# seceq/zkir

Measured on AMD Instinct MI355X. Metric: trace rows/sec (2^20-cycle fib: execution-trace fill + BabyBear NTT/LDE + Poseidon2 Merkle commitment), higher is better.
Workload: dtype u32 (Baby Bear, 31-bit modular) / u64 trace words

## Files before the change

### zkir_amd/csrc/poseidon2.h

```cpp
#pragma once
#include "babybear.h"

#ifndef P2_RF_UNROLL
#define P2_RF_UNROLL 1
#endif
namespace p2 {

constexpr int T = 12, RF = 8, RP = 22, RATE = 8, DIGEST = 4;

struct Consts {
  uint32_t ext[RF][T];
  uint32_t in[RP];
  uint32_t diag[T];
  uint32_t pre[RF][T];
  uint32_t ext0_s[T];
  uint64_t pre_b[RF][T];
  uint32_t in_scale;
  uint32_t out_scale;
  uint32_t carry;
  int32_t in0_neg;
  int32_t pr_c[RP];
  uint64_t pr_a[RP];
  uint64_t pr_k[T];
};

inline uint64_t splitmix64(uint64_t& s) {
  uint64_t z = (s += 0x9E3779B97F4A7C15ull);
  z = (z ^ (z >> 30)) * 0xBF58476D1CE4E5B9ull;
  z = (z ^ (z >> 27)) * 0x94D049BB133111EBull;
  return z ^ (z >> 31);
}

inline void ext_matrix_inverse(uint32_t inv[T][T]) {
  static const uint32_t M4[4][4] = {{5, 7, 1, 3}, {4, 6, 1, 1}, {1, 3, 5, 7}, {1, 1, 4, 6}};
  uint32_t a[T][2 * T];
  for (int i = 0; i < T; i++)
    for (int j = 0; j < T; j++) {
      a[i][j] = M4[i & 3][j & 3] * ((i >> 2) == (j >> 2) ? 2u : 1u);
      a[i][T + j] = i == j;
    }
  for (int col = 0; col < T; col++) {
    int piv = col;
    while (a[piv][col] == 0) piv++;
    for (int j = 0; j < 2 * T; j++) { const uint32_t t = a[col][j]; a[col][j] = a[piv][j]; a[piv][j] = t; }
    const uint32_t pinv = bb::inv(a[col][col]);
    for (int j = 0; j < 2 * T; j++) a[col][j] = bb::mul(a[col][j], pinv);
    for (int i = 0; i < T; i++) {
      if (i == col || a[i][col] == 0) continue;
      const uint32_t f = a[i][col];
      for (int j = 0; j < 2 * T; j++) a[i][j] = bb::sub(a[i][j], bb::mul(f, a[col][j]));
    }
  }
  for (int i = 0; i < T; i++) for (int j = 0; j < T; j++) inv[i][j] = a[i][T + j];
}

inline void generate(Consts& c) {
  uint64_t s = 0x5A4B49522D50322Dull;
  auto next = [&]() -> uint32_t { for (;;) { const uint32_t v = (uint32_t)(splitmix64(s) >> 33); if (v < bb::P) return bb::to_mont(v); } };
  for (int r = 0; r < RF; r++) for (int i = 0; i < T; i++) c.ext[r][i] = next();
  for (int r = 0; r < RP; r++) c.in[r] = next();
  c.diag[0] = bb::to_mont(bb::P - 2);
  for (int i = 1; i < T; i++) c.diag[i] = bb::to_mont(1u << (i - 1));
  uint32_t minv[T][T];
  ext_matrix_inverse(minv);
  for (int r = 0; r < RF; r++)
    for (int i = 0; i < T; i++) {
      uint32_t v = 0;
      if (r != RF / 2 - 1 && r != RF - 1)
        for (int j = 0; j < T; j++) v = bb::add(v, bb::mul(minv[i][j], bb::from_mont(c.ext[r + 1][j])));
      c.pre[r][i] = bb::to_mont(bb::to_mont(v));
    }
  {
    constexpr uint64_t INV7 = 1725656503ull;
    const uint32_t R = bb::R1, Rinv = bb::inv(R);
    const uint32_t R6 = bb::pow(R, 6);
    uint32_t g[RF + 1], h[RF];
    g[RF / 2] = R;
    for (int r = RF / 2 - 1; r >= 0; r--) { h[r] = bb::mul(g[r + 1], R); g[r] = bb::pow(bb::mul(h[r], R6), INV7); }
    {
      uint32_t f[RP], hx[RP];
      for (int r = 0; r < RP; r++) { f[r] = r < 3 ? R : bb::mul(f[r - 3], Rinv); hx[r] = bb::pow(bb::mul(f[r], R6), INV7); }
      const uint32_t G = bb::mul(f[RP - 1], Rinv), R2c = bb::mul(R, R);
      for (int r = 0; r < RP; r++) {
        const uint32_t hn = r + 1 < RP ? hx[r + 1] : G, rcn = bb::from_mont(r + 1 < RP ? c.in[r + 1] : c.ext[RF / 2][0]);
        c.pr_c[r] = (int32_t)bb::mul(bb::mul(hn, R2c), bb::inv(f[r]));
        c.pr_a[r] = bb::mul(bb::mul(hn, rcn), R);
      }
      c.pr_k[0] = 0;
      for (int i = 1; i < T; i++) c.pr_k[i] = bb::mul(f[RP - 1], bb::from_mont(c.ext[RF / 2][i]));
      g[RF / 2] = G;
    }
    for (int r = RF / 2; r < RF; r++) { h[r] = bb::mul(bb::pow(g[r], 7), bb::inv(R6)); g[r + 1] = bb::mul(h[r], Rinv); }
    const uint32_t f_in = bb::mul(g[0], R), f_out = g[RF];
    for (int i = 0; i < T; i++) c.ext0_s[i] = bb::mul(bb::from_mont(c.ext[0][i]), f_in);
    for (int r = 0; r < RF; r++)
      for (int i = 0; i < T; i++) {
        uint32_t v = 0;
        if (r != RF / 2 - 1 && r != RF - 1)
          for (int j = 0; j < T; j++) v = bb::add(v, bb::mul(minv[i][j], bb::from_mont(c.ext[r + 1][j])));
        c.pre_b[r][i] = ((uint64_t)bb::P << 32) | bb::mul(bb::mul(v, h[r]), R);
      }
    c.in_scale = bb::mul(f_in, R);
    c.out_scale = bb::mul(R, bb::inv(f_out));
    c.carry = bb::mul(bb::mul(f_in, R), bb::inv(f_out));
    c.in0_neg = (int32_t)c.in[0] - (int32_t)bb::P;
  }
}

BB_HD uint32_t sbox_lazy(uint32_t x, uint32_t addend = 0) {
  const uint32_t x2 = bb::mont_mul_lazy(x, x), x3 = bb::mont_mul(x2, x), x6 = bb::mont_mul_lazy(x3, x3);
  return bb::mont_mul_add_lazy(x6, x, addend);
}
BB_HD uint32_t sbox(uint32_t x) { return bb::reduce_2p(sbox_lazy(x)); }

BB_HD void m4_wide(uint32_t a, uint32_t b, uint32_t c, uint32_t d, uint64_t* y) {
#if defined(P2_ZEXT_MAD) && defined(__HIP_DEVICE_COMPILE__)
  uint64_t za, zc;
  asm("v_mad_u64_u32 %0, vcc, %1, 1, 0" : "=v"(za) : "v"(a) : "vcc");
  asm("v_mad_u64_u32 %0, vcc, %1, 1, 0" : "=v"(zc) : "v"(c) : "vcc");
  const uint64_t t0 = bb::mad_wide<1>(za, b), t1 = bb::mad_wide<1>(zc, d);
#else
  const uint64_t t0 = bb::acc_add(a, b), t1 = bb::acc_add(c, d);
#endif
  const uint64_t t2 = bb::mad_wide<2>(t1, b), t3 = bb::mad_wide<2>(t0, d);
  const uint64_t t4 = (t1 << 2) + t3, t5 = (t0 << 2) + t2;
  y[0] = t3 + t5; y[1] = t5; y[2] = t2 + t4; y[3] = t4;
}
template <bool ADD_RC>
BB_HD void ext_linear(uint32_t* s, const uint32_t* rc) {
  uint64_t y[T];
// ... 88 lines not shown
  uint64_t acc = (uint64_t)w[1];
#pragma unroll
  for (int i = 2; i < T; i++) acc += (uint64_t)w[i];
  const int64_t sum = bb::sacc_add((int64_t)acc, s0);
  x = int_next_x(smad<-2>(sum, s0), c, r);
#pragma unroll
  for (int i = 1; i < T; i++) w[i] = (int64_t)(((uint64_t)w[i] << (i - 1)) + (uint64_t)sum);
}
constexpr uint64_t lazy_rounds_bound(uint64_t start, int rounds) {
  uint64_t b[T] = {}, top = 0;
  for (int i = 1; i < T; i++) b[i] = start;
  for (int r = 0; r < rounds; r++) {
    uint64_t sum = bb::P;
    for (int i = 1; i < T; i++) sum += b[i];
    if (sum + 2 * (uint64_t)bb::P > top) top = sum + 2 * (uint64_t)bb::P;
    for (int i = 1; i < T; i++) { b[i] = sum + (b[i] << (i - 1)); if (b[i] > top) top = b[i]; }
  }
  return top;
}
constexpr uint64_t lazy_reduced_bound(uint64_t acc) { return (acc >> 32) + bb::P / 2 + 2; }
static_assert(lazy_rounds_bound(1ull << 31, 3) < (1ull << 62), "three partial rounds on words below 2^31 stay inside what a Montgomery reduction takes");
static_assert(lazy_reduced_bound(lazy_rounds_bound(1ull << 31, 3)) <= (1ull << 31), ".. and their reduction is a word below 2^31 again");
static_assert(lazy_reduced_bound(lazy_rounds_bound(1ull << 31, 1) + bb::P) < bb::P, "the words leave the last round (one round + the next full round's constant) inside (-p, p)");
BB_HD void int_rounds_scaled(uint32_t* s, const Consts& c) {
  int32_t x = (int32_t)s[0] + c.in0_neg;
  int32_t t[T];
  int64_t w[T];
#pragma unroll
  for (int i = 1; i < T; i++) t[i] = (int32_t)s[i];
#pragma unroll 1
  for (int r = 0; r < RP - 1; r += 3) {
    int_round_a(x, t, w, c, r);
    int_round_w(x, w, c, r + 1);
    int_round_w(x, w, c, r + 2);
#pragma unroll
    for (int i = 1; i < T; i++) t[i] = bb::smont_reduce_wide(w[i]);
  }
  int_round_a(x, t, w, c, RP - 1);
  s[0] = (uint32_t)x;
#pragma unroll
  for (int i = 1; i < T; i++) s[i] = (uint32_t)bb::smont_reduce_wide((int64_t)((uint64_t)w[i] + c.pr_k[i]));
}
BB_HD void permute_scaled(uint32_t* s, const Consts& c) {
  ext_linear_scaled<true>(s, c.ext0_s);
#pragma unroll P2_RF_UNROLL
  for (int r = 0; r < RF / 2; r++) {
#pragma unroll
    for (int i = 0; i < T; i++) s[i] = sbox_biased(s[i], c.pre_b[r][i]);
    ext_linear_scaled<false>(s, nullptr);
  }
  int_rounds_scaled(s, c);
#pragma unroll P2_RF_UNROLL
  for (int r = RF / 2; r < RF; r++) {
#pragma unroll
    for (int i = 0; i < T; i++) s[i] = sbox_biased(s[i], c.pre_b[r][i]);
    ext_linear_scaled<false>(s, nullptr);
  }
}

#if defined(__HIPCC__)
template <int CTRL>
__device__ __forceinline__ uint32_t quad_perm(uint32_t v) { return (uint32_t)__builtin_amdgcn_mov_dpp((int)v, CTRL, 0xF, 0xF, true); }
template <int CTRL>
__device__ __forceinline__ uint64_t quad_perm64(uint64_t v) { return ((uint64_t)quad_perm<CTRL>((uint32_t)(v >> 32)) << 32) | quad_perm<CTRL>((uint32_t)v); }

template <bool ADD_RC>
__device__ __forceinline__ void ext_linear_quad_scaled(uint32_t* s, const uint32_t* m4row, const uint32_t* rc) {
  uint64_t y[3];
#pragma unroll
  for (int b = 0; b < 3; b++) {
    const uint32_t v0 = quad_perm<0x00>(s[b]), v1 = quad_perm<0x55>(s[b]), v2 = quad_perm<0xAA>(s[b]), v3 = quad_perm<0xFF>(s[b]);
    y[b] = (uint64_t)v0 * m4row[0] + (uint64_t)v1 * m4row[1] + (uint64_t)v2 * m4row[2] + (uint64_t)v3 * m4row[3];
  }
  const uint64_t sum = y[0] + y[1] + y[2];
#pragma unroll
  for (int b = 0; b < 3; b++) {
    uint64_t v = y[b] + sum;
    if (ADD_RC) v += rc[b];
    s[b] = bb::mont_reduce_wide(v);
  }
// ... 108 lines not shown
```

### zkir_amd/csrc/stark.hip

```cpp
#include <hip/hip_runtime.h>

#include <array>
#include <atomic>
#include <chrono>
#include <cstdio>
#include <cstdlib>
#include <cstddef>
#include <memory>
#include <mutex>
#include <vector>

#include "../../include/zkir_amd.h"
#include "../../include/zkir_amd_experimental.h"
#include "air.h"
#include "babybear.h"
#include "host.h"
#include "hashcall.h"
#include "poseidon2.h"
#include "verify_stages.h"

namespace {

constexpr int NT = 256;

// ... 413 lines not shown
}


__global__ __launch_bounds__(NT) void selector_inverse_kernel(uint32_t log_n, const uint32_t* __restrict__ tw_fwd, uint32_t* __restrict__ inv_xm1) {
  const uint32_t N2 = 2u << log_n, N = N2 >> 1;
  const uint32_t j0 = (blockIdx.x * NT + threadIdx.x) * 8;
  if (j0 >= N2) return;
  uint32_t d[8], pre[8];
  uint32_t run = bb::R1;
#pragma unroll
  for (int k = 0; k < 8; k++) {
    const uint32_t j = j0 + k;
    const uint32_t wj = j < N ? tw_fwd[j] : bb::neg(tw_fwd[j - N]);
    d[k] = bb::sub(bb::mont_mul(wj, bb::to_mont(bb::GEN)), bb::R1);
    pre[k] = run; run = bb::mont_mul(run, d[k]);
  }
  uint32_t inv = bb::R1, b = run, e = bb::P - 2;
  while (e) { if (e & 1) inv = bb::mont_mul(inv, b); b = bb::mont_mul(b, b); e >>= 1; }
#pragma unroll
  for (int k = 7; k >= 0; k--) { inv_xm1[j0 + k] = bb::mont_mul(inv, pre[k]); inv = bb::mont_mul(inv, d[k]); }
}


__global__ __launch_bounds__(NT) void leaf_hash_kernel(const p2::Consts* __restrict__ cp, const uint32_t* __restrict__ mat, uint32_t width, uint64_t n, uint32_t in_scale, uint32_t* __restrict__ digests) {
  const uint64_t j = (uint64_t)blockIdx.x * NT + threadIdx.x;
  if (j >= n) return;
  uint32_t s[p2::T];
#pragma unroll
  for (int i = 0; i < p2::T; i++) s[i] = 0;
  const uint4* m4 = reinterpret_cast<const uint4*>(mat);
  const uint32_t carry = cp->carry, out_scale = cp->out_scale;
  for (uint32_t off = 0; off < width; off += p2::RATE) {
    const uint4 lo = m4[((uint64_t)(off >> 3) * n + j) * 2], hi = m4[((uint64_t)(off >> 3) * n + j) * 2 + 1];
    const uint32_t v[8] = {lo.x, lo.y, lo.z, lo.w, hi.x, hi.y, hi.z, hi.w};
#pragma unroll
    for (int i = 0; i < p2::RATE; i++) s[i] = off + i < width ? bb::mont_mul_lazy(v[i], in_scale) : bb::mont_mul_lazy(s[i], carry);
#pragma unroll
    for (int i = p2::RATE; i < p2::T; i++) s[i] = bb::mont_mul_lazy(s[i], carry);
    p2::permute_scaled(s, *cp);
  }
  if (width == 0) p2::permute_scaled(s, *cp);
  uint4 d = make_uint4(bb::mont_mul(s[0], out_scale), bb::mont_mul(s[1], out_scale), bb::mont_mul(s[2], out_scale), bb::mont_mul(s[3], out_scale));
  reinterpret_cast<uint4*>(digests)[j] = d;
}

__global__ __launch_bounds__(NT) void leaf_absorb_kernel(const p2::Consts* __restrict__ cp, const uint32_t* __restrict__ mat, uint32_t width, uint32_t b0, uint32_t b1, uint64_t n, uint32_t in_scale,
                                                         uint4* __restrict__ state, int first, int last, uint32_t* __restrict__ digests) {
  const uint64_t j = (uint64_t)blockIdx.x * NT + threadIdx.x;
  if (j >= n) return;
  uint32_t s[p2::T];
  if (first) {
#pragma unroll
    for (int i = 0; i < p2::T; i++) s[i] = 0;
  } else {
    const uint4 a = state[j], b = state[n + j], c = state[2 * n + j];
    s[0] = a.x; s[1] = a.y; s[2] = a.z; s[3] = a.w; s[4] = b.x; s[5] = b.y; s[6] = b.z; s[7] = b.w; s[8] = c.x; s[9] = c.y; s[10] = c.z; s[11] = c.w;
  }
  const uint4* m4 = reinterpret_cast<const uint4*>(mat);
  const uint32_t carry = cp->carry, out_scale = cp->out_scale;
  for (uint32_t blk = b0; blk < b1; blk++) {
    const uint32_t off = blk * 8;
    const uint4 lo = m4[((uint64_t)blk * n + j) * 2], hi = m4[((uint64_t)blk * n + j) * 2 + 1];
    const uint32_t v[8] = {lo.x, lo.y, lo.z, lo.w, hi.x, hi.y, hi.z, hi.w};
#pragma unroll
    for (int i = 0; i < p2::RATE; i++) s[i] = off + i < width ? bb::mont_mul_lazy(v[i], in_scale) : bb::mont_mul_lazy(s[i], carry);
#pragma unroll
    for (int i = p2::RATE; i < p2::T; i++) s[i] = bb::mont_mul_lazy(s[i], carry);
    p2::permute_scaled(s, *cp);
  }
  if (last) {
    reinterpret_cast<uint4*>(digests)[j] = make_uint4(bb::mont_mul(s[0], out_scale), bb::mont_mul(s[1], out_scale), bb::mont_mul(s[2], out_scale), bb::mont_mul(s[3], out_scale));
  } else {
    state[j] = make_uint4(s[0], s[1], s[2], s[3]); state[n + j] = make_uint4(s[4], s[5], s[6], s[7]); state[2 * n + j] = make_uint4(s[8], s[9], s[10], s[11]);
  }
}

__global__ __launch_bounds__(NT) void compress_kernel(const p2::Consts* __restrict__ cp, const uint32_t* __restrict__ in, uint64_t n_out, uint32_t* __restrict__ out) {
  const uint64_t i = (uint64_t)blockIdx.x * NT + threadIdx.x;
  if (i >= n_out) return;
  const uint4 l = reinterpret_cast<const uint4*>(in)[2 * i], r = reinterpret_cast<const uint4*>(in)[2 * i + 1];
  const uint32_t k = cp->in_scale, ko = cp->out_scale;
  uint32_t s[p2::T] = {bb::mont_mul_lazy(l.x, k), bb::mont_mul_lazy(l.y, k), bb::mont_mul_lazy(l.z, k), bb::mont_mul_lazy(l.w, k), bb::mont_mul_lazy(r.x, k), bb::mont_mul_lazy(r.y, k),
                       bb::mont_mul_lazy(r.z, k), bb::mont_mul_lazy(r.w, k), 0, 0, 0, 0};
  p2::permute_scaled(s, *cp);
  reinterpret_cast<uint4*>(out)[i] = make_uint4(bb::mont_mul(s[0], ko), bb::mont_mul(s[1], ko), bb::mont_mul(s[2], ko), bb::mont_mul(s[3], ko));
}

constexpr uint32_t SUBTREE = 1024, NT_SUB = 1024;
__global__ __launch_bounds__(NT_SUB) void subtree_kernel(const p2::Consts* __restrict__ cp, uint32_t* cur, uint64_t m, uint32_t per_wg, uint32_t* counter) {
  __shared__ uint4 buf[SUBTREE];
  __shared__ uint32_t last_one;
  const uint32_t t = threadIdx.x;
  uint64_t pos0 = (uint64_t)blockIdx.x * per_wg;
  for (uint32_t e = t; e < per_wg; e += NT_SUB) {
    const uint4 v = reinterpret_cast<const uint4*>(cur)[pos0 + e];
    buf[e] = make_uint4(bb::to_mont(v.x), bb::to_mont(v.y), bb::to_mont(v.z), bb::to_mont(v.w));
  }
  __syncthreads();
 levels:
  for (uint32_t cnt = per_wg; cnt > 1; cnt >>= 1) {
    cur += 4 * m; m >>= 1; pos0 >>= 1;
    const uint32_t n_perm = cnt / 2;
    if (n_perm > NT_SUB / 16) {
      const bool active = t < n_perm;
      uint32_t s[p2::T];
      if (active) {
        const uint4 l = buf[2 * t], r = buf[2 * t + 1];
        const uint32_t k_in = bb::from_mont(cp->in_scale);
        s[0] = bb::mont_mul_lazy(l.x, k_in); s[1] = bb::mont_mul_lazy(l.y, k_in); s[2] = bb::mont_mul_lazy(l.z, k_in); s[3] = bb::mont_mul_lazy(l.w, k_in);
        s[4] = bb::mont_mul_lazy(r.x, k_in); s[5] = bb::mont_mul_lazy(r.y, k_in); s[6] = bb::mont_mul_lazy(r.z, k_in); s[7] = bb::mont_mul_lazy(r.w, k_in);
        s[8] = s[9] = s[10] = s[11] = 0;
      }
      __syncthreads();
      if (active) {
        p2::permute_scaled(s, *cp);
        const uint32_t ko = cp->out_scale, ko_m = bb::to_mont(ko);
        buf[t] = make_uint4(bb::mont_mul(s[0], ko_m), bb::mont_mul(s[1], ko_m), bb::mont_mul(s[2], ko_m), bb::mont_mul(s[3], ko_m));
        reinterpret_cast<uint4*>(cur)[pos0 + t] = make_uint4(bb::mont_mul(s[0], ko), bb::mont_mul(s[1], ko), bb::mont_mul(s[2], ko), bb::mont_mul(s[3], ko));
      }
    } else {
      const uint32_t pi = t >> 4, l = t & 15;
      const bool active = pi < n_perm;
      const uint32_t* words = reinterpret_cast<const uint32_t*>(buf);
      uint32_t s = 0;
      if (active && l < 8) s = bb::mont_mul_lazy(words[8 * pi + l], bb::from_mont(cp->in_scale));
      __syncthreads();
      if (active) {
        s = p2::permute_row16_scaled(s, (int)l, *cp);
        if (l < 4) {
          const uint32_t ko = cp->out_scale;
          reinterpret_cast<uint32_t*>(buf)[4 * pi + l] = bb::mont_mul(s, bb::to_mont(ko));
          cur[4 * (pos0 + pi) + l] = bb::mont_mul(s, ko);
        }
      }
    }
    __syncthreads();
  }
#if defined(__HIP_DEVICE_COMPILE__) && !defined(__gfx950__)
#error "subtree_kernel's hand-over relies on the gfx950 (gfx9) s_waitcnt encoding and on vmcnt covering stores"
#endif
  if (m > 1) {
    if (t < 4) {
      const uint32_t v = reinterpret_cast<const uint32_t*>(buf)[t];
      __hip_atomic_store(&cur[4 * pos0 + t], bb::from_mont(v), __ATOMIC_RELAXED, __HIP_MEMORY_SCOPE_AGENT);
      asm volatile("" ::: "memory");
      __builtin_amdgcn_s_waitcnt(0x0F70);
      asm volatile("" ::: "memory");
    }
    if (t == 0) {
      const uint32_t done = __hip_atomic_fetch_add(counter, 1u, __ATOMIC_RELAXED, __HIP_MEMORY_SCOPE_AGENT);
      asm volatile("" ::: "memory");
      last_one = done == (uint32_t)m - 1;
      if (last_one) __hip_atomic_store(counter, 0u, __ATOMIC_RELAXED, __HIP_MEMORY_SCOPE_AGENT);
    }
    __syncthreads();
    if (!last_one) return;
    asm volatile("" ::: "memory");
    per_wg = (uint32_t)m; pos0 = 0;
    for (uint32_t e = t; e < 4 * per_wg; e += NT_SUB)
      reinterpret_cast<uint32_t*>(buf)[e] = bb::to_mont(__hip_atomic_load(&cur[e], __ATOMIC_RELAXED, __HIP_MEMORY_SCOPE_AGENT));
    __syncthreads();
    goto levels;
  }
}

__global__ __launch_bounds__(NT) void modmul_peak_kernel(uint32_t* __restrict__ out, uint32_t iters) {
  uint32_t a[8], c[8];
#pragma unroll
  for (int k = 0; k < 8; k++) { a[k] = (threadIdx.x * 2654435761u + blockIdx.x * 40503u + k * 7919u) % bb::P; c[k] = (a[k] * 31u + 7u) % bb::P; }
  for (uint32_t i = 0; i < iters; i++) {
#pragma unroll
    for (int k = 0; k < 8; k++) a[k] = bb::mont_mul_lazy(a[k], c[k]);
  }
  uint32_t r = 0;
#pragma unroll
  for (int k = 0; k < 8; k++) r ^= a[k];
  if (r == 0xFFFFFFFFu && iters == 0xFFFFFFFFu) out[0] = r;
}

constexpr uint32_t SYNC_SLOTS = 1024;
struct SyncRing {
  uint32_t* d_slots = nullptr;
  std::atomic<uint32_t> next{0};
// ... 23 lines not shown
  uint32_t* d_g_lo = nullptr;
  uint32_t* d_g_lo_m = nullptr;
  uint32_t* d_inv_xm1 = nullptr;
  uint32_t* d_g_hi = nullptr;
  uint32_t* d_small_inv = nullptr;
  uint32_t* d_small_fwd = nullptr;
  p2::Consts consts;
  p2::Consts* d_p2 = nullptr;
  mutable hipStream_t ov_stream = nullptr; mutable hipEvent_t ov_ev[2] = {nullptr, nullptr}; mutable std::vector<hipEvent_t> ov_group_ev; mutable uint4* d_ov_state = nullptr; mutable size_t ov_state_bytes = 0;
  mutable SyncRing sync;
  mutable std::mutex mu;
  mutable unsigned char* arena = nullptr;
  mutable size_t arena_size = 0, arena_off = 0;
  mutable zkir::HostPin pin;
};

namespace {
int lde_launch(const zkir_stark_ctx* c, uint32_t* in, uint32_t width, uint32_t* out, bool mont_out, hipStream_t s) {
  const zkir::LdeTables t{(int)c->log_n, c->d_tw_inv, c->d_tw_fwd, mont_out ? c->d_g_lo_m : c->d_g_lo, c->d_g_hi, c->d_small_inv, c->d_small_fwd};
  zkir::lde_run(t, in, (width + 7) / 8, out, s);
  return check_launch("lde");
}
int merkle_commit(const zkir_stark_ctx* c, const uint32_t* mat, uint32_t width, uint64_t n_leaves, uint32_t* tree, bool mont_in, hipStream_t s) {
  hipLaunchKernelGGL(leaf_hash_kernel, dim3(grid_for(n_leaves)), dim3(NT), 0, s, c->d_p2, mat, width, n_leaves, mont_in ? bb::from_mont(c->consts.in_scale) : c->consts.in_scale, tree);
  launch_tree_levels(c->d_p2, tree, n_leaves, c->sync, s);
  return check_launch("merkle_commit");
}
}

extern "C" {

uint32_t zkir_main_trace_width(void) { return air::committed_width(false); }
uint32_t zkir_main_trace_width_for(uint32_t deferred) { return air::committed_width((int)deferred); }

void zkir_poseidon2_permute(uint32_t state[12]) {
  static const p2::Consts consts = [] { p2::Consts c; p2::generate(c); return c; }();
  uint32_t s[p2::T];
  for (int i = 0; i < p2::T; i++) s[i] = bb::to_mont(state[i] % bb::P);
  p2::permute(s, consts);
  for (int i = 0; i < p2::T; i++) state[i] = bb::from_mont(s[i]);
}

void zkir_poseidon2_permute_scaled(uint32_t state[12], uint32_t rounds) {
  static const p2::Consts consts = [] { p2::Consts c; p2::generate(c); return c; }();
  uint32_t s[p2::T];
  for (int i = 0; i < p2::T; i++) s[i] = bb::mont_mul_lazy(state[i] % bb::P, consts.in_scale);
  for (uint32_t r = 0; r < rounds; r++) {
// ... 46 lines not shown
  uint32_t* d = nullptr;
  if (hipMalloc(&d, 256) != hipSuccess) return 0.0;
  const uint32_t blocks = 256 * 16, iters = 4096;
  hipEvent_t a, b;
  (void)hipEventCreate(&a); (void)hipEventCreate(&b);
  hipLaunchKernelGGL(modmul_peak_kernel, dim3(blocks), dim3(NT), 0, s, d, 64u);
  (void)hipEventRecord(a, s);
  hipLaunchKernelGGL(modmul_peak_kernel, dim3(blocks), dim3(NT), 0, s, d, iters);
  (void)hipEventRecord(b, s);
  (void)hipEventSynchronize(b);
  float ms = 0;
  (void)hipEventElapsedTime(&ms, a, b);
  (void)hipEventDestroy(a); (void)hipEventDestroy(b); (void)hipFree(d);
  return ms > 0 ? (double)blocks * NT * iters * 8.0 / (ms * 1e-3) : 0.0;
}

int zkir_stark_ctx_create(uint32_t log_n, uint32_t log_blowup, zkir_stark_ctx** out) {
  if (!out || log_n < 1 || log_n > 26 || log_blowup != 1) { zkir::set_last_error({ZKIR_ERR_ARGUMENT, "zkir_stark_ctx_create: need 1 <= log_n <= 26 and log_blowup == 1"}); return ZKIR_ERR_ARGUMENT; }
  *out = nullptr;
  zkir_stark_ctx* c = new zkir_stark_ctx();
  c->log_n = log_n; c->log_blowup = log_blowup;
  const uint32_t N = 1u << log_n;
  const uint32_t n_inv = N >= 2 ? N / 2 : 1, n_hi = (N >> 10) + 1;
  p2::generate(c->consts);
  hipError_t e = hipMalloc((void**)&c->d_p2, sizeof(p2::Consts));
  if (e == hipSuccess) e = hipMemcpy(c->d_p2, &c->consts, sizeof(p2::Consts), hipMemcpyHostToDevice);
  if (e == hipSuccess) e = hipMalloc(&c->sync.d_slots, SYNC_SLOTS * sizeof(uint32_t));
  if (e == hipSuccess) e = hipMemset(c->sync.d_slots, 0, SYNC_SLOTS * sizeof(uint32_t));
  if (e == hipSuccess) e = hipMalloc(&c->d_tw_inv, (size_t)n_inv * 4);
  if (e == hipSuccess) e = hipMalloc(&c->d_tw_fwd, (size_t)N * 4);
  if (e == hipSuccess) e = hipMalloc(&c->d_g_lo, 1024 * 4);
  if (e == hipSuccess) e = hipMalloc(&c->d_g_hi, (size_t)n_hi * 4);
  if (e == hipSuccess) e = hipMalloc(&c->d_g_lo_m, 1024 * 4);
  if (e == hipSuccess) e = hipMalloc(&c->d_inv_xm1, (size_t)2 * N * 4);
  const int Bm = log_n < 10 ? (int)log_n : 10;
  const uint32_t n_si = Bm >= 1 ? (1u << (Bm - 1)) : 1, n_sf = 1u << Bm;
  if (e == hipSuccess) e = hipMalloc(&c->d_small_inv, (size_t)n_si * 4);
  if (e == hipSuccess) e = hipMalloc(&c->d_small_fwd, (size_t)n_sf * 4);
  if (e != hipSuccess) { zkir::set_last_error({ZKIR_ERR_DEVICE, std::string("zkir_stark_ctx_create: ") + hipGetErrorString(e)}); zkir_stark_ctx_free(c); return ZKIR_ERR_DEVICE; }
  const uint32_t wN = bb::root_of_unity(log_n), w2N = bb::root_of_unity(log_n + 1);
  hipLaunchKernelGGL(powers_kernel, dim3(grid_for(n_inv)), dim3(NT), 0, 0, bb::inv(wN), bb::R1, c->d_tw_inv, n_inv);
  hipLaunchKernelGGL(powers_kernel, dim3(grid_for(N)), dim3(NT), 0, 0, w2N, bb::R1, c->d_tw_fwd, N);
  hipLaunchKernelGGL(powers_kernel, dim3(4), dim3(NT), 0, 0, bb::GEN, bb::to_mont(bb::inv(N % bb::P)), c->d_g_lo, 1024u);
  hipLaunchKernelGGL(powers_kernel, dim3(4), dim3(NT), 0, 0, bb::GEN, bb::to_mont(bb::to_mont(bb::inv(N % bb::P))), c->d_g_lo_m, 1024u);
  hipLaunchKernelGGL(powers_kernel, dim3(grid_for(n_hi)), dim3(NT), 0, 0, bb::pow(bb::GEN, 1024), bb::R1, c->d_g_hi, n_hi);
  hipLaunchKernelGGL(selector_inverse_kernel, dim3(grid_for((2ull * N + 7) / 8)), dim3(NT), 0, 0, log_n, c->d_tw_fwd, c->d_inv_xm1);
  hipLaunchKernelGGL(powers_kernel, dim3(grid_for(n_si)), dim3(NT), 0, 0, bb::inv(bb::root_of_unity(Bm)), bb::R1, c->d_small_inv, n_si);
  hipLaunchKernelGGL(powers_kernel, dim3(grid_for(n_sf)), dim3(NT), 0, 0, bb::root_of_unity(Bm + 1), bb::R1, c->d_small_fwd, n_sf);
  if (hipDeviceSynchronize() != hipSuccess || check_launch("stark ctx tables") != ZKIR_OK) { zkir_stark_ctx_free(c); return ZKIR_ERR_DEVICE; }
// ... 137 lines not shown
  const zkir::LdeTables t{(int)c->log_n, c->d_tw_inv, c->d_tw_fwd, c->d_g_lo, c->d_g_hi, c->d_small_inv, c->d_small_fwd};
  (void)hipEventRecord(c->ov_ev[0], s); (void)hipStreamWaitEvent(c->ov_stream, c->ov_ev[0], 0);
  for (uint32_t g = 0; g < n_groups; g++) {
    const uint32_t b0 = g * group, b1 = std::min(nb, b0 + group);
    zkir::lde_run(t, in + (uint64_t)b0 * N * 8, b1 - b0, out + (uint64_t)b0 * N2 * 8, s);
    (void)hipEventRecord(c->ov_group_ev[g], s); (void)hipStreamWaitEvent(c->ov_stream, c->ov_group_ev[g], 0);
    hipLaunchKernelGGL(leaf_absorb_kernel, dim3(grid_for(N2)), dim3(NT), 0, c->ov_stream, c->d_p2, out, width, b0, b1, N2, c->consts.in_scale, c->d_ov_state, g == 0 ? 1 : 0, g + 1 == n_groups ? 1 : 0, tree);
  }
  (void)hipEventRecord(c->ov_ev[1], c->ov_stream); (void)hipStreamWaitEvent(s, c->ov_ev[1], 0);
  launch_tree_levels(c->d_p2, tree, N2, c->sync, s);
  return check_launch("commit_overlapped");
}

int zkir_lde_launch(const zkir_stark_ctx* c, uint32_t* in, uint32_t width, uint32_t* out, void* stream) { return lde_launch(c, in, width, out, false, (hipStream_t)stream); }

int zkir_merkle_commit_launch(const zkir_stark_ctx* c, const uint32_t* mat, uint32_t width, uint64_t n_leaves, uint32_t* tree, void* stream) {
  hipStream_t s = (hipStream_t)stream;
  if (!c || n_leaves == 0 || (n_leaves & (n_leaves - 1))) { zkir::set_last_error({ZKIR_ERR_ARGUMENT, "merkle: null context, or n_leaves not a power of two"}); return ZKIR_ERR_ARGUMENT; }
  return merkle_commit(c, mat, width, n_leaves, tree, false, s);
}

int zkir_merkle_leaves_launch(const zkir_stark_ctx* c, const uint32_t* mat, uint32_t width, uint64_t n_leaves, uint32_t* digests, void* stream) {
  if (!c || !mat || !digests || n_leaves == 0) { zkir::set_last_error({ZKIR_ERR_ARGUMENT, "merkle leaves: null argument or no leaves"}); return ZKIR_ERR_ARGUMENT; }
  hipLaunchKernelGGL(leaf_hash_kernel, dim3(grid_for(n_leaves)), dim3(NT), 0, (hipStream_t)stream, c->d_p2, mat, width, n_leaves, c->consts.in_scale, digests);
  return check_launch("merkle_leaves");
}

int zkir_merkle_cap_launch(const zkir_stark_ctx* c, uint32_t* tree, uint64_t n_digests, void* stream) {
  if (!c || n_digests == 0 || (n_digests & (n_digests - 1))) { zkir::set_last_error({ZKIR_ERR_ARGUMENT, "merkle cap: null context, or n_digests not a power of two"}); return ZKIR_ERR_ARGUMENT; }
  launch_tree_levels(c->d_p2, tree, n_digests, c->sync, (hipStream_t)stream);
  return check_launch("merkle_cap");
}

}

#include "stark_prove.inl"
```

Measured before the change: 196.1 million.

## Fold Poseidon2 input scaling into per-domain constant sets and prune dead sponge lanes

Builds three Poseidon2 constant sets (scaled, canonical-input, Montgomery-input). Each set folds the input scaling into the round constants and the first-round factors, so leaf hashing and compression no longer multiply every input word by a scale. A new sponge path precomputes the capacity lanes for zero-capacity compression, skips the reductions of dead output lanes in the last linear layer, and merges the entry constant of the partial rounds into one multiply-add. It also drops the to_mont/from_mont conversions in the subtree kernel and adds an occupancy hint to the leaf and compress kernels. The cost is three times the device constant memory and more complex constant derivation, which brings a correctness risk.

```diff
diff --git a/zkir_amd/csrc/poseidon2.h b/zkir_amd/csrc/poseidon2.h
--- a/zkir_amd/csrc/poseidon2.h
+++ b/zkir_amd/csrc/poseidon2.h
@@ -22,7 +22,13 @@
   int32_t pr_c[RP];
   uint64_t pr_a[RP];
   uint64_t pr_k[T];
+  int32_t x0_mul;
+  uint64_t x0_add;
+  uint32_t rc_in[T];
+  uint64_t rc_car[T];
+  uint64_t cap0_y[4];
 };
+constexpr int SET_SCALED = 0, SET_CANON = 1, SET_MONT = 2, N_SETS = 3;
 
 inline uint64_t splitmix64(uint64_t& s) {
   uint64_t z = (s += 0x9E3779B97F4A7C15ull);
@@ -54,14 +60,13 @@
   for (int i = 0; i < T; i++) for (int j = 0; j < T; j++) inv[i][j] = a[i][T + j];
 }
 
-inline void generate(Consts& c) {
+inline void generate_rounds(Consts& c, uint32_t minv[T][T]) {
   uint64_t s = 0x5A4B49522D50322Dull;
   auto next = [&]() -> uint32_t { for (;;) { const uint32_t v = (uint32_t)(splitmix64(s) >> 33); if (v < bb::P) return bb::to_mont(v); } };
   for (int r = 0; r < RF; r++) for (int i = 0; i < T; i++) c.ext[r][i] = next();
   for (int r = 0; r < RP; r++) c.in[r] = next();
   c.diag[0] = bb::to_mont(bb::P - 2);
   for (int i = 1; i < T; i++) c.diag[i] = bb::to_mont(1u << (i - 1));
-  uint32_t minv[T][T];
   ext_matrix_inverse(minv);
   for (int r = 0; r < RF; r++)
     for (int i = 0; i < T; i++) {
@@ -70,42 +75,67 @@
         for (int j = 0; j < T; j++) v = bb::add(v, bb::mul(minv[i][j], bb::from_mont(c.ext[r + 1][j])));
       c.pre[r][i] = bb::to_mont(bb::to_mont(v));
     }
+}
+constexpr uint64_t INV7 = 1725656503ull;
+inline void generate_factors(Consts& c, uint32_t f_in, const uint32_t minv[T][T]) {
+  const uint32_t R = bb::R1, Rinv = bb::inv(R);
+  const uint32_t R6 = bb::pow(R, 6), R6inv = bb::inv(R6);
+  uint32_t g[RF + 1], h[RF];
+  g[0] = bb::mul(f_in, Rinv);
+  for (int r = 0; r < RF / 2; r++) { h[r] = bb::mul(bb::pow(g[r], 7), R6inv); g[r + 1] = bb::mul(h[r], Rinv); }
   {
-    constexpr uint64_t INV7 = 1725656503ull;
-    const uint32_t R = bb::R1, Rinv = bb::inv(R);
-    const uint32_t R6 = bb::pow(R, 6);
-    uint32_t g[RF + 1], h[RF];
-    g[RF / 2] = R;
-    for (int r = RF / 2 - 1; r >= 0; r--) { h[r] = bb::mul(g[r + 1], R); g[r] = bb::pow(bb::mul(h[r], R6), INV7); }
-    {
-      uint32_t f[RP], hx[RP];
-      for (int r = 0; r < RP; r++) { f[r] = r < 3 ? R : bb::mul(f[r - 3], Rinv); hx[r] = bb::pow(bb::mul(f[r], R6), INV7); }
-      const uint32_t G = bb::mul(f[RP - 1], Rinv), R2c = bb::mul(R, R);
-      for (int r = 0; r < RP; r++) {
-        const uint32_t hn = r + 1 < RP ? hx[r + 1] : G, rcn = bb::from_mont(r + 1 < RP ? c.in[r + 1] : c.ext[RF / 2][0]);
-        c.pr_c[r] = (int32_t)bb::mul(bb::mul(hn, R2c), bb::inv(f[r]));
-        c.pr_a[r] = bb::mul(bb::mul(hn, rcn), R);
-      }
-      c.pr_k[0] = 0;
-      for (int i = 1; i < T; i++) c.pr_k[i] = bb::mul(f[RP - 1], bb::from_mont(c.ext[RF / 2][i]));
-      g[RF / 2] = G;
-    }
-    for (int r = RF / 2; r < RF; r++) { h[r] = bb::mul(bb::pow(g[r], 7), bb::inv(R6)); g[r + 1] = bb::mul(h[r], Rinv); }
-    const uint32_t f_in = bb::mul(g[0], R), f_out = g[RF];
-    for (int i = 0; i < T; i++) c.ext0_s[i] = bb::mul(bb::from_mont(c.ext[0][i]), f_in);
-    for (int r = 0; r < RF; r++)
-      for (int i = 0; i < T; i++) {
-        uint32_t v = 0;
-        if (r != RF / 2 - 1 && r != RF - 1)
-          for (int j = 0; j < T; j++) v = bb::add(v, bb::mul(minv[i][j], bb::from_mont(c.ext[r + 1][j])));
-        c.pre_b[r][i] = ((uint64_t)bb::P << 32) | bb::mul(bb::mul(v, h[r]), R);
-      }
-    c.in_scale = bb::mul(f_in, R);
-    c.out_scale = bb::mul(R, bb::inv(f_out));
-    c.carry = bb::mul(bb::mul(f_in, R), bb::inv(f_out));
-    c.in0_neg = (int32_t)c.in[0] - (int32_t)bb::P;
-  }
-}
+    uint32_t f[RP], hx[RP];
+    const uint32_t f0 = g[RF / 2];
+    for (int r = 0; r < RP; r++) { f[r] = r < 3 ? f0 : bb::mul(f[r - 3], Rinv); hx[r] = bb::pow(bb::mul(f[r], R6), INV7); }
+    const uint32_t G = bb::mul(f[RP - 1], Rinv), R2c = bb::mul(R, R);
+    for (int r = 0; r < RP; r++) {
+      const uint32_t hn = r + 1 < RP ? hx[r + 1] : G, rcn = bb::from_mont(r + 1 < RP ? c.in[r + 1] : c.ext[RF / 2][0]);
+      c.pr_c[r] = (int32_t)bb::mul(bb::mul(hn, R2c), bb::inv(f[r]));
+      c.pr_a[r] = bb::mul(bb::mul(hn, rcn), R);
+    }
+    c.pr_k[0] = 0;
+    for (int i = 1; i < T; i++) c.pr_k[i] = bb::mul(f[RP - 1], bb::from_mont(c.ext[RF / 2][i]));
+    c.x0_mul = (int32_t)bb::mul(bb::mul(hx[0], R), bb::inv(f0));
+    c.x0_add = bb::mul(bb::mul(hx[0], bb::from_mont(c.in[0])), R);
+    g[RF / 2] = G;
+  }
+  for (int r = RF / 2; r < RF; r++) { h[r] = bb::mul(bb::pow(g[r], 7), R6inv); g[r + 1] = bb::mul(h[r], Rinv); }
+  const uint32_t f_out = g[RF];
+  for (int i = 0; i < T; i++) c.ext0_s[i] = bb::mul(bb::from_mont(c.ext[0][i]), f_in);
+  for (int r = 0; r < RF; r++)
+    for (int i = 0; i < T; i++) {
+      uint32_t v = 0;
+      if (r != RF / 2 - 1 && r != RF - 1)
+        for (int j = 0; j < T; j++) v = bb::add(v, bb::mul(minv[i][j], bb::from_mont(c.ext[r + 1][j])));
+      c.pre_b[r][i] = ((uint64_t)bb::P << 32) | bb::mul(bb::mul(v, h[r]), R);
+    }
+  c.in_scale = bb::mul(f_in, R);
+  c.out_scale = bb::mul(R, bb::inv(f_out));
+  c.carry = bb::mul(bb::mul(f_in, R), bb::inv(f_out));
+  c.in0_neg = (int32_t)c.in[0] - (int32_t)bb::P;
+  for (int i = 0; i < T; i++) {
+    uint32_t v = 0;
+    for (int j = 0; j < T; j++) v = bb::add(v, bb::mul(minv[i][j], bb::from_mont(c.ext[0][j])));
+    c.rc_in[i] = bb::mul(v, f_in);
+    c.rc_car[i] = bb::mul(c.rc_in[i], R);
+  }
+  const uint64_t a = c.rc_in[8], b = c.rc_in[9], cc = c.rc_in[10], d = c.rc_in[11];
+  c.cap0_y[0] = 5 * a + 7 * b + cc + 3 * d; c.cap0_y[1] = 4 * a + 6 * b + cc + d; c.cap0_y[2] = a + 3 * b + 5 * cc + 7 * d; c.cap0_y[3] = a + b + 4 * cc + 6 * d;
+}
+inline void generate(Consts& c) {
+  uint32_t minv[T][T];
+  generate_rounds(c, minv);
+  const uint32_t R = bb::R1, R6 = bb::pow(R, 6);
+  uint32_t g = R;
+  for (int r = RF / 2 - 1; r >= 0; r--) g = bb::pow(bb::mul(bb::mul(g, R), R6), INV7);
+  generate_factors(c, bb::mul(g, R), minv);
+}
+inline void generate_for(Consts& c, uint32_t f_in) {
+  uint32_t minv[T][T];
+  generate_rounds(c, minv);
+  generate_factors(c, f_in, minv);
+}
+inline void generate_sets(Consts* sets) { generate(sets[SET_SCALED]); generate_for(sets[SET_CANON], 1u); generate_for(sets[SET_MONT], bb::R1); }
 
 BB_HD uint32_t sbox_lazy(uint32_t x, uint32_t addend = 0) {
   const uint32_t x2 = bb::mont_mul_lazy(x, x), x3 = bb::mont_mul(x2, x), x6 = bb::mont_mul_lazy(x3, x3);
@@ -240,8 +270,11 @@
 static_assert(lazy_rounds_bound(1ull << 31, 3) < (1ull << 62), "three partial rounds on words below 2^31 stay inside what a Montgomery reduction takes");
 static_assert(lazy_reduced_bound(lazy_rounds_bound(1ull << 31, 3)) <= (1ull << 31), ".. and their reduction is a word below 2^31 again");
 static_assert(lazy_reduced_bound(lazy_rounds_bound(1ull << 31, 1) + bb::P) < bb::P, "the words leave the last round (one round + the next full round's constant) inside (-p, p)");
+static_assert((((uint64_t)bb::P + 128) * bb::P + bb::P) < ((uint64_t)bb::P << 31), "the entry product of word 0 is inside what a signed Montgomery product takes");
+static_assert(((((uint64_t)bb::P + 128) * bb::P + bb::P) >> 32) + bb::P / 2 + 2 < bb::P, ".. and leaves |x| < p, inside the S-box input bound |x| <= p + 128");
+template <bool ENTRY_MUL = false>
 BB_HD void int_rounds_scaled(uint32_t* s, const Consts& c) {
-  int32_t x = (int32_t)s[0] + c.in0_neg;
+  int32_t x = ENTRY_MUL ? bb::smont_mul_add((int32_t)s[0], c.x0_mul, c.x0_add) : (int32_t)s[0] + c.in0_neg;
   int32_t t[T];
   int64_t w[T];
 #pragma unroll
@@ -267,13 +300,133 @@
     for (int i = 0; i < T; i++) s[i] = sbox_biased(s[i], c.pre_b[r][i]);
     ext_linear_scaled<false>(s, nullptr);
   }
-  int_rounds_scaled(s, c);
+  int_rounds_scaled<false>(s, c);
 #pragma unroll P2_RF_UNROLL
   for (int r = RF / 2; r < RF; r++) {
 #pragma unroll
     for (int i = 0; i < T; i++) s[i] = sbox_biased(s[i], c.pre_b[r][i]);
     ext_linear_scaled<false>(s, nullptr);
   }
+}
+
+enum Live { LIVE_ALL, LIVE_CAP, LIVE_DIGEST };
+template <bool ZERO_CAP>
+BB_HD void ext_linear_first(uint32_t* s, const Consts& c) {
+  uint64_t y[T];
+  m4_wide(s[0], s[1], s[2], s[3], y); m4_wide(s[4], s[5], s[6], s[7], y + 4);
+  if (ZERO_CAP) {
+#pragma unroll
+    for (int j = 0; j < 4; j++) y[8 + j] = c.cap0_y[j];
+  } else m4_wide(s[8], s[9], s[10], s[11], y + 8);
+  uint64_t sum[4];
+#pragma unroll
+  for (int j = 0; j < 4; j++) sum[j] = y[j] + y[4 + j] + y[8 + j];
+#pragma unroll
+  for (int k = 0; k < T; k++) s[k] = bb::mont_reduce_wide(y[k] + sum[k & 3]);
+}
+BB_HD void dead4(uint32_t* s) {
+#if defined(__HIP_DEVICE_COMPILE__)
+  asm("" : "=v"(s[0]), "=v"(s[1]), "=v"(s[2]), "=v"(s[3]));
+#else
+  s[0] = s[1] = s[2] = s[3] = 0;
+#endif
+}
+BB_HD Live uniform(Live l) {
+#if defined(__HIP_DEVICE_COMPILE__)
+  uint32_t v = (uint32_t)l;
+  asm("" : "+s"(v));
+  return (Live)v;
+#else
+  return l;
+#endif
+}
+BB_HD void ext_linear_live(uint32_t* s, Live live) {
+  uint64_t y[T];
+  m4_wide(s[0], s[1], s[2], s[3], y); m4_wide(s[4], s[5], s[6], s[7], y + 4); m4_wide(s[8], s[9], s[10], s[11], y + 8);
+  uint64_t sum[4];
+#pragma unroll
+  for (int j = 0; j < 4; j++) sum[j] = y[j] + y[4 + j] + y[8 + j];
+  if (live == LIVE_ALL) {
+#pragma unroll
+    for (int k = 0; k < T; k++) s[k] = bb::mont_reduce_wide(y[k] + sum[k & 3]);
+  } else if (live == LIVE_CAP) {
+#pragma unroll
+    for (int k = RATE; k < T; k++) s[k] = bb::mont_reduce_wide(y[k] + sum[k & 3]);
+    dead4(s); dead4(s + 4);
+  } else {
+#pragma unroll
+    for (int k = 0; k < DIGEST; k++) s[k] = bb::mont_reduce_wide(y[k] + sum[k & 3]);
+    dead4(s + 4); dead4(s + 8);
+  }
+}
+template <bool ZERO_CAP>
+BB_HD void sponge_rounds(uint32_t* s, const Consts& c, Live live) {
+  ext_linear_first<ZERO_CAP>(s, c);
+#pragma unroll P2_RF_UNROLL
+  for (int r = 0; r < RF / 2; r++) {
+#pragma unroll
+    for (int i = 0; i < T; i++) s[i] = sbox_biased(s[i], c.pre_b[r][i]);
+    ext_linear_scaled<false>(s, nullptr);
+  }
+  int_rounds_scaled<true>(s, c);
+#pragma unroll P2_RF_UNROLL
+  for (int r = RF / 2; r < RF; r++) {
+#pragma unroll
+    for (int i = 0; i < T; i++) s[i] = sbox_biased(s[i], c.pre_b[r][i]);
+    ext_linear_live(s, r < RF - 1 ? LIVE_ALL : live);
+  }
+}
+template <Live LIVE, bool ZERO_CAP>
+BB_HD void permute_sponge(uint32_t* s, const Consts& c) { sponge_rounds<ZERO_CAP>(s, c, uniform(LIVE)); }
+BB_HD void sponge_absorb(uint32_t* s, const uint32_t* x, const Consts& c) {
+#pragma unroll
+  for (int i = 0; i < RATE; i++) s[i] = x[i] + c.rc_in[i];
+}
+BB_HD uint32_t sponge_keep(uint32_t s, const Consts& c, int i) { return bb::mont_mul_add_lazy(s, c.carry, c.rc_car[i]); }
+BB_HD const Consts& fresh(const Consts& c) {
+  uint32_t z = 0;
+#if defined(__HIP_DEVICE_COMPILE__)
+  asm volatile("" : "+s"(z));
+#endif
+  return (&c)[z];
+}
+template <class Load>
+BB_HD void sponge_hash(const Consts& c, uint32_t width, Load&& load, uint32_t* digest) {
+  const uint32_t nb = (width + RATE - 1) / RATE, rag = width % RATE;
+  uint32_t s[T];
+  uint32_t b = 0;
+  do {
+    uint32_t v[RATE] = {0, 0, 0, 0, 0, 0, 0, 0};
+    const Consts& k = fresh(c);
+    const bool ragged = rag && b + 1 == nb;
+    if (b < nb) load(b, v);
+    if (b == 0) {
+      const uint32_t n0 = nb == 0 ? 0u : ragged ? rag : (uint32_t)RATE;
+#pragma unroll
+      for (int i = 0; i < RATE; i++) s[i] = ((uint32_t)i < n0 ? v[i] : 0u) + k.rc_in[i];
+#pragma unroll
+      for (int i = RATE; i < T; i++) s[i] = k.rc_in[i];
+    } else {
+      if (ragged) {
+#pragma unroll
+        for (int i = 0; i < RATE; i++) s[i] = (uint32_t)i < rag ? v[i] + k.rc_in[i] : sponge_keep(s[i], k, i);
+      } else sponge_absorb(s, v, k);
+#pragma unroll
+      for (int i = RATE; i < T; i++) s[i] = sponge_keep(s[i], k, i);
+    }
+    sponge_rounds<false>(s, k, b + 1 >= nb ? LIVE_DIGEST : rag && b + 2 == nb ? LIVE_ALL : LIVE_CAP);
+  } while (++b < nb);
+#pragma unroll
+  for (int i = 0; i < DIGEST; i++) digest[i] = bb::mont_mul(s[i], c.out_scale);
+}
+BB_HD void sponge_compress(const Consts& c, const uint32_t* x, uint32_t* digest) {
+  uint32_t s[T];
+  sponge_absorb(s, x, c);
+#pragma unroll
+  for (int i = RATE; i < T; i++) s[i] = 0;
+  permute_sponge<LIVE_DIGEST, true>(s, c);
+#pragma unroll
+  for (int i = 0; i < DIGEST; i++) digest[i] = bb::mont_mul(s[i], c.out_scale);
 }
 
 #if defined(__HIPCC__)
diff --git a/zkir_amd/csrc/stark.hip b/zkir_amd/csrc/stark.hip
--- a/zkir_amd/csrc/stark.hip
+++ b/zkir_amd/csrc/stark.hip
@@ -459,26 +459,17 @@
 }
 
 
-__global__ __launch_bounds__(NT) void leaf_hash_kernel(const p2::Consts* __restrict__ cp, const uint32_t* __restrict__ mat, uint32_t width, uint64_t n, uint32_t in_scale, uint32_t* __restrict__ digests) {
+constexpr int P2_WAVES = 8;
+__global__ __launch_bounds__(NT, P2_WAVES) void leaf_hash_kernel(const p2::Consts* __restrict__ cp, const uint32_t* __restrict__ mat, uint32_t width, uint64_t n, uint32_t* __restrict__ digests) {
   const uint64_t j = (uint64_t)blockIdx.x * NT + threadIdx.x;
   if (j >= n) return;
-  uint32_t s[p2::T];
-#pragma unroll
-  for (int i = 0; i < p2::T; i++) s[i] = 0;
   const uint4* m4 = reinterpret_cast<const uint4*>(mat);
-  const uint32_t carry = cp->carry, out_scale = cp->out_scale;
-  for (uint32_t off = 0; off < width; off += p2::RATE) {
-    const uint4 lo = m4[((uint64_t)(off >> 3) * n + j) * 2], hi = m4[((uint64_t)(off >> 3) * n + j) * 2 + 1];
-    const uint32_t v[8] = {lo.x, lo.y, lo.z, lo.w, hi.x, hi.y, hi.z, hi.w};
-#pragma unroll
-    for (int i = 0; i < p2::RATE; i++) s[i] = off + i < width ? bb::mont_mul_lazy(v[i], in_scale) : bb::mont_mul_lazy(s[i], carry);
-#pragma unroll
-    for (int i = p2::RATE; i < p2::T; i++) s[i] = bb::mont_mul_lazy(s[i], carry);
-    p2::permute_scaled(s, *cp);
-  }
-  if (width == 0) p2::permute_scaled(s, *cp);
-  uint4 d = make_uint4(bb::mont_mul(s[0], out_scale), bb::mont_mul(s[1], out_scale), bb::mont_mul(s[2], out_scale), bb::mont_mul(s[3], out_scale));
-  reinterpret_cast<uint4*>(digests)[j] = d;
+  uint32_t d[p2::DIGEST];
+  p2::sponge_hash(*cp, width, [&](uint32_t b, uint32_t* v) {
+    const uint4 lo = m4[((uint64_t)b * n + j) * 2], hi = m4[((uint64_t)b * n + j) * 2 + 1];
+    v[0] = lo.x; v[1] = lo.y; v[2] = lo.z; v[3] = lo.w; v[4] = hi.x; v[5] = hi.y; v[6] = hi.z; v[7] = hi.w;
+  }, d);
+  reinterpret_cast<uint4*>(digests)[j] = make_uint4(d[0], d[1], d[2], d[3]);
 }
 
 __global__ __launch_bounds__(NT) void leaf_absorb_kernel(const p2::Consts* __restrict__ cp, const uint32_t* __restrict__ mat, uint32_t width, uint32_t b0, uint32_t b1, uint64_t n, uint32_t in_scale,
@@ -512,15 +503,14 @@
   }
 }
 
-__global__ __launch_bounds__(NT) void compress_kernel(const p2::Consts* __restrict__ cp, const uint32_t* __restrict__ in, uint64_t n_out, uint32_t* __restrict__ out) {
+__global__ __launch_bounds__(NT, P2_WAVES) void compress_kernel(const p2::Consts* __restrict__ cp, const uint32_t* __restrict__ in, uint64_t n_out, uint32_t* __restrict__ out) {
   const uint64_t i = (uint64_t)blockIdx.x * NT + threadIdx.x;
   if (i >= n_out) return;
   const uint4 l = reinterpret_cast<const uint4*>(in)[2 * i], r = reinterpret_cast<const uint4*>(in)[2 * i + 1];
-  const uint32_t k = cp->in_scale, ko = cp->out_scale;
-  uint32_t s[p2::T] = {bb::mont_mul_lazy(l.x, k), bb::mont_mul_lazy(l.y, k), bb::mont_mul_lazy(l.z, k), bb::mont_mul_lazy(l.w, k), bb::mont_mul_lazy(r.x, k), bb::mont_mul_lazy(r.y, k),
-                       bb::mont_mul_lazy(r.z, k), bb::mont_mul_lazy(r.w, k), 0, 0, 0, 0};
-  p2::permute_scaled(s, *cp);
-  reinterpret_cast<uint4*>(out)[i] = make_uint4(bb::mont_mul(s[0], ko), bb::mont_mul(s[1], ko), bb::mont_mul(s[2], ko), bb::mont_mul(s[3], ko));
+  const uint32_t x[p2::RATE] = {l.x, l.y, l.z, l.w, r.x, r.y, r.z, r.w};
+  uint32_t d[p2::DIGEST];
+  p2::sponge_compress(cp[p2::SET_CANON], x, d);
+  reinterpret_cast<uint4*>(out)[i] = make_uint4(d[0], d[1], d[2], d[3]);
 }
 
 constexpr uint32_t SUBTREE = 1024, NT_SUB = 1024;
@@ -530,8 +520,7 @@
   const uint32_t t = threadIdx.x;
   uint64_t pos0 = (uint64_t)blockIdx.x * per_wg;
   for (uint32_t e = t; e < per_wg; e += NT_SUB) {
-    const uint4 v = reinterpret_cast<const uint4*>(cur)[pos0 + e];
-    buf[e] = make_uint4(bb::to_mont(v.x), bb::to_mont(v.y), bb::to_mont(v.z), bb::to_mont(v.w));
+    buf[e] = reinterpret_cast<const uint4*>(cur)[pos0 + e];
   }
   __syncthreads();
  levels:
@@ -540,34 +529,32 @@
     const uint32_t n_perm = cnt / 2;
     if (n_perm > NT_SUB / 16) {
       const bool active = t < n_perm;
-      uint32_t s[p2::T];
+      uint32_t x[p2::RATE];
       if (active) {
         const uint4 l = buf[2 * t], r = buf[2 * t + 1];
-        const uint32_t k_in = bb::from_mont(cp->in_scale);
-        s[0] = bb::mont_mul_lazy(l.x, k_in); s[1] = bb::mont_mul_lazy(l.y, k_in); s[2] = bb::mont_mul_lazy(l.z, k_in); s[3] = bb::mont_mul_lazy(l.w, k_in);
-        s[4] = bb::mont_mul_lazy(r.x, k_in); s[5] = bb::mont_mul_lazy(r.y, k_in); s[6] = bb::mont_mul_lazy(r.z, k_in); s[7] = bb::mont_mul_lazy(r.w, k_in);
-        s[8] = s[9] = s[10] = s[11] = 0;
+        x[0] = l.x; x[1] = l.y; x[2] = l.z; x[3] = l.w; x[4] = r.x; x[5] = r.y; x[6] = r.z; x[7] = r.w;
       }
       __syncthreads();
       if (active) {
-        p2::permute_scaled(s, *cp);
-        const uint32_t ko = cp->out_scale, ko_m = bb::to_mont(ko);
-        buf[t] = make_uint4(bb::mont_mul(s[0], ko_m), bb::mont_mul(s[1], ko_m), bb::mont_mul(s[2], ko_m), bb::mont_mul(s[3], ko_m));
-        reinterpret_cast<uint4*>(cur)[pos0 + t] = make_uint4(bb::mont_mul(s[0], ko), bb::mont_mul(s[1], ko), bb::mont_mul(s[2], ko), bb::mont_mul(s[3], ko));
+        uint32_t d[p2::DIGEST];
+        p2::sponge_compress(cp[p2::SET_CANON], x, d);
+        const uint4 v = make_uint4(d[0], d[1], d[2], d[3]);
+        buf[t] = v;
+        reinterpret_cast<uint4*>(cur)[pos0 + t] = v;
       }
     } else {
       const uint32_t pi = t >> 4, l = t & 15;
       const bool active = pi < n_perm;
       const uint32_t* words = reinterpret_cast<const uint32_t*>(buf);
       uint32_t s = 0;
-      if (active && l < 8) s = bb::mont_mul_lazy(words[8 * pi + l], bb::from_mont(cp->in_scale));
+      if (active && l < 8) s = bb::mont_mul_lazy(words[8 * pi + l], cp->in_scale);
       __syncthreads();
       if (active) {
         s = p2::permute_row16_scaled(s, (int)l, *cp);
         if (l < 4) {
-          const uint32_t ko = cp->out_scale;
-          reinterpret_cast<uint32_t*>(buf)[4 * pi + l] = bb::mont_mul(s, bb::to_mont(ko));
-          cur[4 * (pos0 + pi) + l] = bb::mont_mul(s, ko);
+          const uint32_t v = bb::mont_mul(s, cp->out_scale);
+          reinterpret_cast<uint32_t*>(buf)[4 * pi + l] = v;
+          cur[4 * (pos0 + pi) + l] = v;
         }
       }
     }
@@ -579,7 +566,7 @@
   if (m > 1) {
     if (t < 4) {
       const uint32_t v = reinterpret_cast<const uint32_t*>(buf)[t];
-      __hip_atomic_store(&cur[4 * pos0 + t], bb::from_mont(v), __ATOMIC_RELAXED, __HIP_MEMORY_SCOPE_AGENT);
+      __hip_atomic_store(&cur[4 * pos0 + t], v, __ATOMIC_RELAXED, __HIP_MEMORY_SCOPE_AGENT);
       asm volatile("" ::: "memory");
       __builtin_amdgcn_s_waitcnt(0x0F70);
       asm volatile("" ::: "memory");
@@ -595,7 +582,7 @@
     asm volatile("" ::: "memory");
     per_wg = (uint32_t)m; pos0 = 0;
     for (uint32_t e = t; e < 4 * per_wg; e += NT_SUB)
-      reinterpret_cast<uint32_t*>(buf)[e] = bb::to_mont(__hip_atomic_load(&cur[e], __ATOMIC_RELAXED, __HIP_MEMORY_SCOPE_AGENT));
+      reinterpret_cast<uint32_t*>(buf)[e] = __hip_atomic_load(&cur[e], __ATOMIC_RELAXED, __HIP_MEMORY_SCOPE_AGENT);
     __syncthreads();
     goto levels;
   }
@@ -665,7 +652,7 @@
   return check_launch("lde");
 }
 int merkle_commit(const zkir_stark_ctx* c, const uint32_t* mat, uint32_t width, uint64_t n_leaves, uint32_t* tree, bool mont_in, hipStream_t s) {
-  hipLaunchKernelGGL(leaf_hash_kernel, dim3(grid_for(n_leaves)), dim3(NT), 0, s, c->d_p2, mat, width, n_leaves, mont_in ? bb::from_mont(c->consts.in_scale) : c->consts.in_scale, tree);
+  hipLaunchKernelGGL(leaf_hash_kernel, dim3(grid_for(n_leaves)), dim3(NT), 0, s, c->d_p2 + (mont_in ? p2::SET_MONT : p2::SET_CANON), mat, width, n_leaves, tree);
   launch_tree_levels(c->d_p2, tree, n_leaves, c->sync, s);
   return check_launch("merkle_commit");
 }
@@ -758,9 +745,11 @@
   c->log_n = log_n; c->log_blowup = log_blowup;
   const uint32_t N = 1u << log_n;
   const uint32_t n_inv = N >= 2 ? N / 2 : 1, n_hi = (N >> 10) + 1;
-  p2::generate(c->consts);
-  hipError_t e = hipMalloc((void**)&c->d_p2, sizeof(p2::Consts));
-  if (e == hipSuccess) e = hipMemcpy(c->d_p2, &c->consts, sizeof(p2::Consts), hipMemcpyHostToDevice);
+  std::vector<p2::Consts> sets(p2::N_SETS);
+  p2::generate_sets(sets.data());
+  c->consts = sets[p2::SET_SCALED];
+  hipError_t e = hipMalloc((void**)&c->d_p2, sets.size() * sizeof(p2::Consts));
+  if (e == hipSuccess) e = hipMemcpy(c->d_p2, sets.data(), sets.size() * sizeof(p2::Consts), hipMemcpyHostToDevice);
   if (e == hipSuccess) e = hipMalloc(&c->sync.d_slots, SYNC_SLOTS * sizeof(uint32_t));
   if (e == hipSuccess) e = hipMemset(c->sync.d_slots, 0, SYNC_SLOTS * sizeof(uint32_t));
   if (e == hipSuccess) e = hipMalloc(&c->d_tw_inv, (size_t)n_inv * 4);
@@ -944,7 +933,7 @@
 
 int zkir_merkle_leaves_launch(const zkir_stark_ctx* c, const uint32_t* mat, uint32_t width, uint64_t n_leaves, uint32_t* digests, void* stream) {
   if (!c || !mat || !digests || n_leaves == 0) { zkir::set_last_error({ZKIR_ERR_ARGUMENT, "merkle leaves: null argument or no leaves"}); return ZKIR_ERR_ARGUMENT; }
-  hipLaunchKernelGGL(leaf_hash_kernel, dim3(grid_for(n_leaves)), dim3(NT), 0, (hipStream_t)stream, c->d_p2, mat, width, n_leaves, c->consts.in_scale, digests);
+  hipLaunchKernelGGL(leaf_hash_kernel, dim3(grid_for(n_leaves)), dim3(NT), 0, (hipStream_t)stream, c->d_p2 + p2::SET_CANON, mat, width, n_leaves, digests);
   return check_launch("merkle_leaves");
 }
 
```

Result: no change. 197.3 million (median of 6 runs) (+0.6%).
